# fallenshock/SinDDM

Measured on AMD Instinct MI355X. Metric: diffusion steps/sec (finest scale) + imgs/sec full multi-scale sample, 1/2/4/8 GPU, higher is better.
Workload: dtype f32 (3x3 convs: binary16 hi/lo split products -- Winograd-domain GEMMs with all 4 MFMA terms, fp32 accumulate; fp32-equivalent, error vs float64 = the fp32 oracle's: tests/test_gpu_h2.py; everything else fp32); 1 GPU; C3: 6-scale pyramid, T=1000, finest scale 411x512, batch 64 per GPU, dim=160; batch_per_gpu=64, global_batch=64, scale=5, parallelism=independent chains over 1 GPU(s), one all-gather of the images

## Files before the change

sinddm_amd/csrc/sinddm_fwd.hip:

```cpp
#include "conv_mfma.h"
#include "conv_wino4.h"
#include "conv_wh.h"
#include "internal.h"
#include "step_tail.h"
#include "chain_run.h"
#include <type_traits>
namespace sinddm {

ConvProfiler& conv_profiler() {
    static ConvProfiler p;
    return p;
}

__global__ void pack_kernel(const float* __restrict__ params, float* __restrict__ packed, PackArgs a) {
    long long i = (long long)blockIdx.x * blockDim.x + threadIdx.x;
    if (i >= a.total) return;
    int s = 0;
    long long base = 0;
    while (s < a.nseg - 1 && i >= base + a.seg[s].count) { base += a.seg[s].count; ++s; }
    const PackSeg& g = a.seg[s];
    const long long j = i - base;
    float v = 0.0f;
    if (g.kind == 0) {
        const int co_l = (int)(j % g.co_lds);
// ... 23 lines not shown
        const int cb = (int)r;
        const int m = cb * g.mt * 16 + mt * 16 + (lane & 15);
        const int k = ch * 16 + ks * 4 + (lane >> 4);
        const int M = g.transpose ? g.cin : g.cout;
        const int K = g.transpose ? g.cout : g.cin;
        if (m < M && k < K) {
            float gt[3][3];
#pragma unroll
            for (int a = 0; a < 3; ++a)
#pragma unroll
                for (int b2 = 0; b2 < 3; ++b2) {
                    const int tap = a * 3 + b2;
                    gt[a][b2] = g.transpose ? params[g.w + ((long long)k * g.cin + m) * 9 + (8 - tap)]
                                            : params[g.w + ((long long)m * g.cin + k) * 9 + tap];
                }
            const float G[4][3] = {{1.f, 0.f, 0.f}, {0.5f, 0.5f, 0.5f}, {0.5f, -0.5f, 0.5f}, {0.f, 0.f, 1.f}};
            const int fi = xi >> 2, fj = xi & 3;
            float acc = 0.f;
#pragma unroll
            for (int a = 0; a < 3; ++a) {
                float rowv = 0.f;
#pragma unroll
                for (int b2 = 0; b2 < 3; ++b2) rowv += G[fj][b2] * gt[a][b2];
                acc += G[fi][a] * rowv;
            }
            v = fi == 2 ? -acc : acc;
        }
    } else if (g.kind == 4) {
        long long r = j;
        const int slot = (int)(r % 4); r /= 4;
        const int lane = (int)(r % 64); r /= 64;
        const int q8 = (int)(r % 8); r /= 8;
        const int ks = (int)(r % 4); r /= 4;
        const int fi = (int)(r % 4); r /= 4;
        const int ch = (int)(r % g.nch); r /= g.nch;
        const int cb = (int)r;
        const int e = w3_pos_e(q8 * 4 + slot);
        const int mt = e < 0 ? 0 : e / 6, fj = e < 0 ? 0 : e - mt * 6;
        const int m = cb * 80 + mt * 16 + (lane & 15);
        const int k = ch * 16 + ks * 4 + (lane >> 4);
        const int M4 = g.transpose ? g.cin : g.cout, K4 = g.transpose ? g.cout : g.cin;
        if (e >= 0 && m < M4 && k < K4) {
            const double G2[4][3] = {{1., 0., 0.}, {.5, .5, .5}, {.5, -.5, .5}, {0., 0., 1.}};
            const double G4[6][3] = {{1. / 4, 0., 0.}, {-1. / 6, -1. / 6, -1. / 6}, {-1. / 6, 1. / 6, -1. / 6},
                                     {1. / 24, 1. / 12, 1. / 6}, {1. / 24, -1. / 12, 1. / 6}, {0., 0., 1.}};
            double acc = 0.;
#pragma unroll
            for (int a = 0; a < 3; ++a) {
                double rowv = 0.;
#pragma unroll
                for (int b2 = 0; b2 < 3; ++b2)
                    rowv += G4[fj][b2] * (double)(g.transpose ? params[g.w + ((long long)k * g.cin + m) * 9 + (2 - a) * 3 + (2 - b2)]
                                                              : params[g.w + ((long long)m * g.cin + k) * 9 + a * 3 + b2]);
                acc += G2[fi][a] * rowv;
            }
            v = (float)(fi == 2 ? -acc : acc);
        }
    } else if (g.kind == 1) {
        if (j < g.cout) {
            v = params[g.w + j];
            if (g.w2 >= 0) v += params[g.w2 + j];
        }
    }
    packed[g.dst + j] = v;
}

int pack_launch(const float* params, float* packed, const PackArgs& a, hipStream_t st) {
    const int threads = 256;
    const unsigned grid = (unsigned)((a.total + threads - 1) / threads);
    hipLaunchKernelGGL(pack_kernel, dim3(grid), dim3(threads), 0, st, params, packed, a);
    SINDDM_LAUNCH_CHECK();
    return 0;
}

static int pack_forward(const NetPlan& P, const float* params, float* packed, hipStream_t st) {
    PackArgs a{};
    auto add = [&](PackSeg s) { a.seg[a.nseg++] = s; a.total += s.count; };
    for (int l = 0; l < 4; ++l) {
        const BlockPlan& b = P.blk[l];
        pack_add_conv3x3(a, b.c1, 0, b.c1_w, 0);
        pack_add_conv3x3(a, b.c2, 0, b.c2_w, 0);
        if (b.nchr > 0) pack_add_direct(a, b.pk_res, b.res_w, b.cin, b.cout, 1, b.mt, b.coblks, 0);
        pack_add_conv3x3(a, b.c1, 3, b.c1_w, 0);
        pack_add_conv3x3(a, b.c2, 3, b.c2_w, 0);
        PackSeg t{};
        t.kind = 1; t.cout = b.cout; t.count = (long long)b.coblks * b.mt * 16;
        t.dst = b.pk_b1; t.w = b.c1_b; t.w2 = -1;
        add(t);
        t.dst = b.pk_b2; t.w = b.c2_b; t.w2 = b.res_b;
        add(t);
    }
    PackSeg z{};
    z.kind = 2; z.dst = P.pk_zero; z.count = 64;
    add(z);
    int rc = pack_launch(params, packed, a, st);
    if (rc) return rc;
    PackArgs f{};
    for (int l = 0; l < 4; ++l) {
        pack_add_conv3x3(f, P.blk[l].c1, 4, P.blk[l].c1_w, 0);
        pack_add_conv3x3(f, P.blk[l].c2, 4, P.blk[l].c2_w, 0);
    }
    if (f.nseg > 0) {
        rc = pack_launch(params, packed, f, st);
        if (rc) return rc;
    }
    for (int l = 0; l < 4; ++l) {
        rc = wh_pack(P.blk[l].c1, params + P.blk[l].c1_w, packed, 0, st);
        if (!rc) rc = wh_pack(P.blk[l].c2, params + P.blk[l].c2_w, packed, 0, st);
        if (rc) return rc;
    }
    return head_pack_launch(P, params, packed, st);
}

struct CondArgs {
    const float* params;
    const long long* t_dev;
    int t_host;
    int t_step;
    float scale;
    float* out;
    int cond_stride;
    long long tm0_w, tm0_b, tm2_w, tm2_b;
    long long mlp_w[4], mlp_b[4], tr_w[4], tr_b[4];
    int cin[4], coff[4];
    float* cond_vec;
    float* hidden;
    float* emb_out;
    float* mvec_out;
};
static CondArgs cond_args(const NetPlan& P, const float* params) {
    CondArgs ca{};
    ca.params = params; ca.cond_stride = P.cond_stride;
    ca.tm0_w = P.tm0_w; ca.tm0_b = P.tm0_b; ca.tm2_w = P.tm2_w; ca.tm2_b = P.tm2_b;
    for (int l = 0; l < 4; ++l) {
        ca.mlp_w[l] = P.blk[l].mlp_w; ca.mlp_b[l] = P.blk[l].mlp_b;
        ca.tr_w[l] = P.blk[l].tr_w; ca.tr_b[l] = P.blk[l].tr_b;
        ca.cin[l] = P.blk[l].cin; ca.coff[l] = P.blk[l].cond_off;
    }
    return ca;
}

__global__ __launch_bounds__(128) void cond_kernel(CondArgs a) {
    __shared__ float emb[64];
    __shared__ float h1[128];
    __shared__ float cv[32];
    __shared__ float gv[32];
    __shared__ float mv[32];
    const int b = blockIdx.x;
    const int tid = threadIdx.x;
    const float* P = a.params;
    const float tval = a.t_dev ? (float)a.t_dev[b] : (float)(a.t_host + b * a.t_step);
    if (tid < 32) {
        const int i = tid & 15;
        const float f = (float)exp((double)((float)i * -0.6140226914650789f));
        const float x = (tid < 16) ? tval : a.scale;
        const float arg = x * f;
        const int o = (tid < 16) ? 0 : 32;
        emb[o + i] = sinf(arg);
        emb[o + 16 + i] = cosf(arg);
    }
    __syncthreads();
    if (a.emb_out && tid < 64) a.emb_out[(long long)b * 64 + tid] = emb[tid];
    {
        float s = P[a.tm0_b + tid];
        const float* w = P + a.tm0_w + (long long)tid * 64;
#pragma unroll 8
        for (int k = 0; k < 64; ++k) s = fmaf(w[k], emb[k], s);
        if (a.hidden) a.hidden[(long long)b * 128 + tid] = s;
        h1[tid] = gelu_erf(s);
    }
    __syncthreads();
    if (tid < 32) {
        float s = P[a.tm2_b + tid];
        const float* w = P + a.tm2_w + (long long)tid * 128;
#pragma unroll 8
        for (int k = 0; k < 128; ++k) s = fmaf(w[k], h1[k], s);
        cv[tid] = s;
        gv[tid] = gelu_erf(s);
        if (a.cond_vec) a.cond_vec[(long long)b * 32 + tid] = s;
    }
    __syncthreads();
    for (int l = 0; l < 4; ++l) {
        if (tid < 32) {
            float s = P[a.mlp_b[l] + tid];
            const float* w = P + a.mlp_w[l] + (long long)tid * 32;
#pragma unroll 8
            for (int k = 0; k < 32; ++k) s = fmaf(w[k], gv[k], s);
            mv[tid] = s;
            if (a.mvec_out) a.mvec_out[((long long)b * 4 + l) * 32 + tid] = s;
        }
        __syncthreads();
        for (int c = tid; c < a.cin[l]; c += blockDim.x) {
            float s = P[a.tr_b[l] + c];
            const float* w = P + a.tr_w[l] + (long long)c * 32;
#pragma unroll 8
            for (int k = 0; k < 32; ++k) s = fmaf(w[k], mv[k], s);
            a.out[(long long)b * a.cond_stride + a.coff[l] + c] = s;
        }
        __syncthreads();
    }
}

#ifndef DW_RW_
#define DW_RW_ 4
#endif
constexpr int DW_RW = DW_RW_;
constexpr int DW_TH = 4 * DW_RW, DW_TW = 128, DW_RS = DW_TW + 4, DW_HR = DW_TH + 4;
#ifndef DW_NX_
#define DW_NX_ 2
#endif
constexpr int DW_NX = DW_NX_;

__global__ __launch_bounds__(256) void dwconv5_kernel(const float* __restrict__ x, const float* __restrict__ w,
                                                       const float* __restrict__ bias, const float* __restrict__ cond,
                                                       int cond_stride, const float* __restrict__ addt, int flip,
                                                       float* __restrict__ out, int C, int H, int W, int groupsX, int pi,
                                                       int po, float* __restrict__ amax) {
    __shared__ __attribute__((aligned(16))) float tile[DW_NX][DW_HR * DW_RS];
    const int c = blockIdx.y, b = blockIdx.z;
    const int ty = blockIdx.x / groupsX, gxi = blockIdx.x - ty * groupsX;
    const int y0 = ty * DW_TH, xg0 = gxi * (DW_NX * DW_TW);
    const size_t plane = ((size_t)b * C + c) * H * po;
    const float* src = x + ((size_t)b * C + c) * H * pi;
    constexpr int DW_GR = DW_RS / 4;
    constexpr int DW_NG = DW_HR * DW_GR;
    constexpr int DW_LD = (DW_NG + 255) / 256;
    const __amdgpu_buffer_rsrc_t rsx = __builtin_amdgcn_make_buffer_rsrc(const_cast<float*>(src), 0, H * pi * 4, 0x00020000);
    f32x4 stg[DW_NX][DW_LD];
#pragma unroll
    for (int t = 0; t < DW_NX; ++t) {
        const int x0 = xg0 + t * DW_TW;
#pragma unroll
        for (int k = 0; k < DW_LD; ++k) {
            const int i = threadIdx.x + k * 256;
            const int r = i / DW_GR, g = i - r * DW_GR;
            const int gy = y0 + r - 2, gx = x0 + 4 * g - 2;
            const bool rowok = i < DW_NG && x0 < W && gy >= 0 && gy < H;
            const bool left = gx < 0;
            const int off = rowok ? (gy * pi + (left ? 0 : gx)) * 4 : 0x40000000;
            const f32x4 q = __builtin_bit_cast(f32x4, __builtin_amdgcn_raw_buffer_load_b128(rsx, off, 0, 0));
            f32x4 v = left ? f32x4{0.f, 0.f, q[0], q[1]} : q;
#pragma unroll
            for (int e = 0; e < 4; ++e) v[e] = (rowok && gx + e < W) ? v[e] : 0.0f;
            stg[t][k] = v;
        }
    }
#pragma unroll
    for (int t = 0; t < DW_NX; ++t)
#pragma unroll
        for (int k = 0; k < DW_LD; ++k) {
            const int i = threadIdx.x + k * 256;
            if (i < DW_NG) *reinterpret_cast<f32x4*>(&tile[t][i * 4]) = stg[t][k];
        }
    float wk[25];
#pragma unroll
    for (int k = 0; k < 25; ++k) wk[k] = w[c * 25 + (flip ? 24 - k : k)];
    const float add = (bias ? bias[c] : 0.0f) + (cond ? cond[(size_t)b * cond_stride + c] : 0.0f);
    __syncthreads();
    const int lane = threadIdx.x & 63, wv = threadIdx.x >> 6;
    float mx = 0.f;
#pragma unroll
    for (int t = 0; t < DW_NX; ++t) {
        const int x0 = xg0 + t * DW_TW;
        if (x0 >= W) break;
        f32x2 o[DW_RW];
#pragma unroll
        for (int r = 0; r < DW_RW; ++r) o[r] = f32x2{add, add};
#pragma unroll
        for (int dy = 0; dy < DW_RW + 4; ++dy) {
            f32x2 v[5];
            const float* row = &tile[t][(wv * DW_RW + dy) * DW_RS + lane];
#pragma unroll
            for (int dx = 0; dx < 5; ++dx) v[dx] = f32x2{row[dx], row[dx + 64]};
#pragma unroll
            for (int r = 0; r < DW_RW; ++r) {
                const int ky = dy - r;
                if (ky >= 0 && ky < 5) {
#pragma unroll
                    for (int dx = 0; dx < 5; ++dx) o[r] += wk[ky * 5 + dx] * v[dx];
                }
            }
        }
#pragma unroll
        for (int h = 0; h < 2; ++h) {
            const int gx = x0 + lane + 64 * h;
            if (gx < po) {
#pragma unroll
                for (int r = 0; r < DW_RW; ++r) {
                    const int gy = y0 + wv * DW_RW + r;
                    if (gy < H) {
                        const size_t oidx = plane + (size_t)gy * po + gx;
                        const float ov = gx < W ? (addt ? o[r][h] + addt[oidx] : o[r][h]) : 0.0f;
                        mx = fmaxf(mx, fabsf(ov));
                        out[oidx] = ov;
                    }
                }
            }
        }
    }
    if (amax) amax_publish(mx, amax + (size_t)b * AMAX_STRIDE);
}

#ifndef DWR_ROWS_
#define DWR_ROWS_ 12
#endif
constexpr int DWR_ROWS = DWR_ROWS_;

__global__ __launch_bounds__(256) void dwconv5_rows_kernel(const float* __restrict__ x, const float* __restrict__ w,
                                                            const float* __restrict__ bias, const float* __restrict__ cond,
                                                            int cond_stride, const float* __restrict__ addt, int flip,
                                                            float* __restrict__ out, int C, int H, int W, int bandsX, int Wt,
                                                            float* __restrict__ amax) {
    const int c = blockIdx.y, b = blockIdx.z;
    const int by = blockIdx.x / bandsX, bx = blockIdx.x - by * bandsX;
    const int lane = threadIdx.x & 63, wv = threadIdx.x >> 6;
    const int x4 = (bx * 64 + lane) * 4;
    const int y0 = (by * 4 + wv) * DWR_ROWS;
    const size_t plane = ((size_t)b * C + c) * H * W;
    float wk[25];
#pragma unroll
    for (int k = 0; k < 25; ++k) wk[k] = w[c * 25 + (flip ? 24 - k : k)];
    const float add = (bias ? bias[c] : 0.0f) + (cond ? cond[(size_t)b * cond_stride + c] : 0.0f);
    if (y0 >= H) return;
    const __amdgpu_buffer_rsrc_t rsx = __builtin_amdgcn_make_buffer_rsrc(const_cast<float*>(x + plane), 0, H * W * 4, 0x00020000);
    constexpr int OOBI = 0x40000000;
    const bool colok = x4 < W;
    const bool lok = colok && x4 >= 4, rok = colok && x4 + 4 < W;
    f32x4 acc[DWR_ROWS];
#pragma unroll
    for (int r = 0; r < DWR_ROWS; ++r) acc[r] = f32x4{add, add, add, add};
#pragma unroll
    for (int ir = 0; ir < DWR_ROWS + 4; ++ir) {
        const int gy = y0 + ir - 2;
        const bool rowok = gy >= 0 && gy < H;
        const int base = (gy * W + x4) * 4;
        const f32x4 ql = __builtin_bit_cast(f32x4, __builtin_amdgcn_raw_buffer_load_b128(rsx, (rowok && lok) ? base - 16 : OOBI, 0, 0));
        const f32x4 qm = __builtin_bit_cast(f32x4, __builtin_amdgcn_raw_buffer_load_b128(rsx, (rowok && colok) ? base : OOBI, 0, 0));
        const f32x4 qr = __builtin_bit_cast(f32x4, __builtin_amdgcn_raw_buffer_load_b128(rsx, (rowok && rok) ? base + 16 : OOBI, 0, 0));
        const float in[8] = {ql[2], ql[3], qm[0], qm[1], qm[2], qm[3], qr[0], qr[1]};
#pragma unroll
        for (int r = 0; r < DWR_ROWS; ++r) {
            const int ky = ir - r;
            if (ky >= 0 && ky < 5) {
#pragma unroll
                for (int kx = 0; kx < 5; ++kx) {
#pragma unroll
                    for (int cc = 0; cc < 4; ++cc) acc[r][cc] = fmaf(wk[ky * 5 + kx], in[cc + kx], acc[r][cc]);
                }
            }
        }
    }
    float mx = 0.f;
#pragma unroll
    for (int r = 0; r < DWR_ROWS; ++r) {
        const int gy = y0 + r;
        if (colok && gy < H) {
            const size_t o = plane + (size_t)gy * W + x4;
            f32x4 v = acc[r];
            if (addt) v += *reinterpret_cast<const f32x4*>(addt + o);
            if (x4 + 4 > Wt) {
#pragma unroll
                for (int cc = 0; cc < 4; ++cc) v[cc] = x4 + cc < Wt ? v[cc] : 0.0f;
            }
            mx = fmaxf(fmaxf(mx, fmaxf(fabsf(v[0]), fabsf(v[1]))), fmaxf(fabsf(v[2]), fabsf(v[3])));
            *reinterpret_cast<f32x4*>(out + o) = v;
        }
    }
    if (amax) amax_publish(mx, amax + (size_t)b * AMAX_STRIDE);
}

#ifndef SINDDM_DW_ROWS
#define SINDDM_DW_ROWS 1
#endif

int dwconv_launch(const float* x, const float* w, const float* bias, const float* cond, int cond_stride,
                  const float* addt, int flip, float* out, int B, int C, int H, int W, hipStream_t st, int pi, int po,
                  float* amax) {
    if (pi <= 0) pi = W;
    if (po <= 0) po = W;
    if (SINDDM_DW_ROWS && pi % 4 == 0 && po == pi && pi >= 192) {
        const int bandsX = (pi + 255) / 256, bandsY = (H + 4 * DWR_ROWS - 1) / (4 * DWR_ROWS);
        hipLaunchKernelGGL(dwconv5_rows_kernel, dim3(bandsX * bandsY, C, B), dim3(256), 0, st, x, w, bias, cond, cond_stride,
                           addt, flip, out, C, H, pi, bandsX, W, amax);
        SINDDM_LAUNCH_CHECK();
        return 0;
    }
    const int tilesX = (W + DW_TW - 1) / DW_TW, tilesY = (H + DW_TH - 1) / DW_TH;
    const int groupsX = (tilesX + DW_NX - 1) / DW_NX;
    hipLaunchKernelGGL(dwconv5_kernel, dim3(groupsX * tilesY, C, B), dim3(256), 0, st, x, w, bias, cond, cond_stride,
                       addt, flip, out, C, H, W, groupsX, pi, po, amax);
    SINDDM_LAUNCH_CHECK();
    return 0;
}

__global__ __launch_bounds__(256) void conv3x3_c3_gelu_kernel(const float* __restrict__ in, const float* __restrict__ w,
                                                              const float* __restrict__ bias, float* __restrict__ out,
                                                              float* __restrict__ out_pre, int H, int W, int Cout,
                                                              int co_per_block, int Wt, float* __restrict__ amax) {
    const int HW = H * W;
    const int b = blockIdx.y;
    const int co0 = blockIdx.z * co_per_block;
    const int co1 = min(Cout, co0 + co_per_block);
    const int p = blockIdx.x * 256 + threadIdx.x;
    const bool live = p < HW;
    const int pc = live ? p : HW - 1;
    const int y = pc / W, x = pc - y * W;
    const float* src = in + (size_t)b * 3 * HW;
    float v[27];
#pragma unroll
    for (int ci = 0; ci < 3; ++ci)
#pragma unroll
        for (int ky = 0; ky < 3; ++ky)
#pragma unroll
            for (int kx = 0; kx < 3; ++kx) {
                const int gy = y + ky - 1, gx = x + kx - 1;
                const bool ok = gy >= 0 && gy < H && gx >= 0 && gx < W;
                v[ci * 9 + ky * 3 + kx] = ok ? src[(size_t)ci * HW + (size_t)gy * W + gx] : 0.0f;
            }
    float* dst = out + (size_t)b * Cout * HW + pc;
    float* dpre = out_pre ? out_pre + (size_t)b * Cout * HW + pc : nullptr;
    f32x2 vp[13];
#pragma unroll
    for (int j = 0; j < 13; ++j) vp[j] = f32x2{v[2 * j], v[2 * j + 1]};
    auto dot27 = [&](int co) __attribute__((always_inline)) -> float {
        const float* wc = w + co * 27;
        f32x2 acc2{bias[co], 0.f};
#pragma unroll
        for (int j = 0; j < 13; ++j) {
            const f32x2 wp{wc[2 * j], wc[2 * j + 1]};
            acc2 = __builtin_elementwise_fma(vp[j], wp, acc2);
        }
        return fmaf(v[26], wc[26], acc2.x + acc2.y);
    };
    int co = co0;
    float mx = 0.f;
#pragma unroll 2
    for (; co + 1 < co1; co += 2) {
        const f32x2 acc{dot27(co), dot27(co + 1)};
        if (live) {
            if (dpre) {
                dpre[(size_t)co * HW] = acc.x;
                dpre[(size_t)(co + 1) * HW] = acc.y;
            }
            const f32x2 g = gelu_erf2(acc);
            const float g0 = x < Wt ? g.x : 0.0f, g1 = x < Wt ? g.y : 0.0f;
            mx = fmaxf(mx, fmaxf(fabsf(g0), fabsf(g1)));
            dst[(size_t)co * HW] = g0;
            dst[(size_t)(co + 1) * HW] = g1;
        }
    }
    if (co < co1) {
        const float acc = dot27(co);
        if (live) {
            if (dpre) dpre[(size_t)co * HW] = acc;
            const float g0 = x < Wt ? gelu_erf(acc) : 0.0f;
            mx = fmaxf(mx, fabsf(g0));
            dst[(size_t)co * HW] = g0;
        }
    }
    if (amax) amax_publish(mx, amax + (size_t)b * AMAX_STRIDE);
}

__global__ __launch_bounds__(256) void pad_rows_kernel(const float* __restrict__ in, float* __restrict__ out, int H, int W,
                                                       int Wp, long long nrows) {
    const long long q = (long long)blockIdx.x * 256 + threadIdx.x;
    const int qpr = Wp >> 2;
    if (q >= nrows * qpr) return;
    const long long row = q / qpr;
    const int x = (int)(q - row * qpr) * 4;
    f32x4 v;
#pragma unroll
    for (int e = 0; e < 4; ++e) v[e] = x + e < W ? in[row * W + x + e] : 0.0f;
    *reinterpret_cast<f32x4*>(out + row * Wp + x) = v;
}
__global__ __launch_bounds__(256) void final_conv1x1_pitch_kernel(const float* __restrict__ a, const float* __restrict__ w,
                                                                  const float* __restrict__ bias, float* __restrict__ out,
                                                                  int C, int H, int W, int Wp) {
    const int b = blockIdx.y;
    const int qpr = Wp >> 2;
    const int q = blockIdx.x * 256 + threadIdx.x;
    if (q >= H * qpr) return;
    const int y = q / qpr, x = (q - y * qpr) * 4;
    const size_t HWp = (size_t)H * Wp;
    const float* src = a + (size_t)b * C * HWp + (size_t)y * Wp + x;
    f32x4 o0{bias[0], bias[0], bias[0], bias[0]}, o1{bias[1], bias[1], bias[1], bias[1]}, o2{bias[2], bias[2], bias[2], bias[2]};
#pragma unroll 8
    for (int c = 0; c < C; ++c) {
        const f32x4 v = *reinterpret_cast<const f32x4*>(src + (size_t)c * HWp);
        o0 += w[c] * v;
        o1 += w[C + c] * v;
        o2 += w[2 * C + c] * v;
    }
    const size_t HW = (size_t)H * W;
    float* dst = out + (size_t)b * 3 * HW + (size_t)y * W + x;
#pragma unroll
    for (int e = 0; e < 4; ++e) {
        if (x + e < W) {
            dst[e] = o0[e];
            dst[HW + e] = o1[e];
            dst[2 * HW + e] = o2[e];
        }
    }
}
__global__ __launch_bounds__(256) void final_conv1x1_kernel(const float* __restrict__ a, const float* __restrict__ w,
                                                            const float* __restrict__ bias, float* __restrict__ out,
                                                            int C, int HW) {
    const int b = blockIdx.y;
    const int p = (blockIdx.x * 256 + threadIdx.x) * 4;
    if (p >= HW) return;
    const float* src = a + (size_t)b * C * HW + p;
    float* dst = out + (size_t)b * 3 * HW + p;
    if (p + 3 < HW) {
        f32x4 o0{bias[0], bias[0], bias[0], bias[0]}, o1{bias[1], bias[1], bias[1], bias[1]},
            o2{bias[2], bias[2], bias[2], bias[2]};
#pragma unroll 8
        for (int c = 0; c < C; ++c) {
            const f32x4 v = *reinterpret_cast<const f32x4*>(src + (size_t)c * HW);
            o0 += w[c] * v;
            o1 += w[C + c] * v;
            o2 += w[2 * C + c] * v;
        }
        *reinterpret_cast<f32x4*>(dst) = o0;
        *reinterpret_cast<f32x4*>(dst + HW) = o1;
        *reinterpret_cast<f32x4*>(dst + 2 * (size_t)HW) = o2;
    } else {
        for (int j = 0; p + j < HW; ++j) {
            float o0 = bias[0], o1 = bias[1], o2 = bias[2];
            for (int c = 0; c < C; ++c) {
                const float v = src[(size_t)c * HW + j];
                o0 = fmaf(w[c], v, o0);
                o1 = fmaf(w[C + c], v, o1);
                o2 = fmaf(w[2 * C + c], v, o2);
            }
            dst[j] = o0;
            dst[HW + j] = o1;
            dst[2 * (size_t)HW + j] = o2;
        }
    }
}

enum { Q_FUSE_GX = 1,
       Q_FUSE_CAX = 2 };
enum { Q_ROUND_QUAD = 0, Q_ROUND_QUAD_UN4 = Q_FUSE_GX, Q_ROUND_FLOAT = Q_FUSE_GX | Q_FUSE_CAX };

__device__ __forceinline__ float q_fma(float a, float b, float c) { return __builtin_fmaf(a, b, c); }
__device__ __forceinline__ f32x4 q_fma(float a, f32x4 b, f32x4 c) { return __builtin_elementwise_fma(f32x4{a, a, a, a}, b, c); }

template <typename T>
__device__ __forceinline__ T q_sample_elem(const T& x, const T& o, const T& z, bool mix, float g, float ca, float cb, int r) {
    T v = x;
    if (mix) v = (r & Q_FUSE_GX) ? q_fma(g, v, (1.0f - g) * o) : q_fma(1.0f - g, o, g * v);
    return (r & Q_FUSE_CAX) ? q_fma(ca, v, cb * z) : q_fma(cb, z, ca * v);
}

template <int VEC, int UN>
__global__ __launch_bounds__(256) void q_sample_kernel(const float* __restrict__ x0, const float* __restrict__ xo,
                                                       const float* __restrict__ nz, float* __restrict__ out,
                                                       const float* __restrict__ tabA, const float* __restrict__ tabB,
                                                       const float* __restrict__ gam, const long long* __restrict__ t_dev,
                                                       int t_host, long long n) {
    const int b = blockIdx.y;
    const long long t = t_dev ? t_dev[b] : (long long)t_host;
    const float ca = tabA[t], cb = tabB[t];
    const float g = (xo != nullptr) ? gam[t] : 0.0f;
    const size_t base = (size_t)b * n;
    if constexpr (VEC == 4) {
        const long long nq = n >> 2;
        const f32x4* x4 = reinterpret_cast<const f32x4*>(x0 + base);
        const f32x4* o4 = xo ? reinterpret_cast<const f32x4*>(xo + base) : nullptr;
        const f32x4* z4 = reinterpret_cast<const f32x4*>(nz + base);
        f32x4* y4 = reinterpret_cast<f32x4*>(out + base);
        for (long long q0 = (long long)blockIdx.x * (256 * UN) + threadIdx.x; q0 < nq; q0 += (long long)gridDim.x * (256 * UN)) {
            f32x4 v[UN], z[UN], o[UN];
#pragma unroll
            for (int u = 0; u < UN; ++u) {
                const long long q = q0 + u * 256;
                const bool ok = q < nq;
                v[u] = ok ? __builtin_nontemporal_load(x4 + q) : f32x4{0.f, 0.f, 0.f, 0.f};
                z[u] = ok ? __builtin_nontemporal_load(z4 + q) : f32x4{0.f, 0.f, 0.f, 0.f};
                if (o4) o[u] = ok ? __builtin_nontemporal_load(o4 + q) : f32x4{0.f, 0.f, 0.f, 0.f};
            }
#pragma unroll
            for (int u = 0; u < UN; ++u) {
                const long long q = q0 + u * 256;
                if (q >= nq) continue;
                y4[q] = q_sample_elem(v[u], o[u], z[u], o4 != nullptr, g, ca, cb, UN == 4 ? Q_ROUND_QUAD_UN4 : Q_ROUND_QUAD);
            }
        }
    } else {
        for (long long i = (long long)blockIdx.x * 256 + threadIdx.x; i < n; i += (long long)gridDim.x * 256) {
            float o;
            if (xo) o = xo[base + i];
            out[base + i] = q_sample_elem(x0[base + i], o, nz[base + i], xo != nullptr, g, ca, cb, Q_ROUND_FLOAT);
        }
    }
}


template <bool WRAP>
__device__ __forceinline__ void upsample_axis(float scale, int dst, int n, int& i0, int& i1, float& lam) {
    float f = fmaf(scale, (float)dst + 0.5f, -0.5f);
    if (WRAP) {
        const float fl = floorf(f);
        lam = f - fl;
        i0 = (int)fl % n;
        if (i0 < 0) i0 += n;
        i1 = i0 + 1 == n ? 0 : i0 + 1;
    } else {
        f = f < 0.0f ? 0.0f : f;
        i0 = (int)f; if (i0 > n - 1) i0 = n - 1;
        i1 = i0 + 1 < n ? i0 + 1 : n - 1;
        lam = f - (float)i0;
    }
}

template <bool WRAP_Y, bool WRAP_X>
__global__ __launch_bounds__(256) void upsample_bilinear_kernel(const float* __restrict__ in, float* __restrict__ out,
                                                                int h, int w, int H, int W, float sy, float sx) {
    const int bc = blockIdx.y;
    const int p = blockIdx.x * 256 + threadIdx.x;
    if (p >= H * W) return;
    const int oy = p / W, ox = p - oy * W;
    int iy0, iy1, ix0, ix1;
    float ly, lx;
    upsample_axis<WRAP_Y>(sy, oy, h, iy0, iy1, ly);
    upsample_axis<WRAP_X>(sx, ox, w, ix0, ix1, lx);
    const float* s = in + (size_t)bc * h * w;
    const float tl = s[iy0 * w + ix0], tr = s[iy0 * w + ix1], bl = s[iy1 * w + ix0], br = s[iy1 * w + ix1];
    out[(size_t)bc * H * W + p] = (1.0f - ly) * ((1.0f - lx) * tl + lx * tr) + ly * ((1.0f - lx) * bl + lx * br);
}

template <int VEC>
__global__ __launch_bounds__(256) void wrap_halo_kernel(float* ext, const float* src, long long nq, int H, int W, int hy,
                                                        int hx) {
    const int He = H + 2 * hy, We = W + 2 * hx, qpr = We / VEC;
    for (long long q = (long long)blockIdx.x * 256 + threadIdx.x; q < nq; q += (long long)gridDim.x * 256) {
        const long long row = q / qpr;
        const int x = (int)(q - row * qpr) * VEC;
        const long long bc = row / He;
        const int y = (int)(row - bc * He);
        if (!src && y >= hy && y < hy + H && x >= hx && x < hx + W) continue;
        int cy = (y - hy) % H, cx = (x - hx) % W;
        if (cy < 0) cy += H;
        if (cx < 0) cx += W;
        const float* s = src ? src + ((size_t)bc * H + cy) * W + cx : ext + ((size_t)bc * He + hy + cy) * We + hx + cx;
        float* d = ext + ((size_t)bc * He + y) * We + x;
        if (VEC == 4) *reinterpret_cast<f32x4*>(d) = *reinterpret_cast<const f32x4*>(s);
        else *d = *s;
    }
}

int wrap_halo_launch(float* ext, const float* src, int BC, int H, int W, int hy, int hx, hipStream_t st) {
    if (hy == 0 && hx == 0 && !src) return 0;
    const bool vec = W % 4 == 0 && hx % 4 == 0 &&
                     ((reinterpret_cast<uintptr_t>(ext) | reinterpret_cast<uintptr_t>(src)) & 15) == 0;
    const long long nq = (long long)BC * (H + 2 * hy) * ((W + 2 * hx) / (vec ? 4 : 1));
    long long bx = (nq + 255) / 256;
    if (bx > 8192) bx = 8192;
    if (vec) hipLaunchKernelGGL(wrap_halo_kernel<4>, dim3((unsigned)bx), dim3(256), 0, st, ext, src, nq, H, W, hy, hx);
    else hipLaunchKernelGGL(wrap_halo_kernel<1>, dim3((unsigned)bx), dim3(256), 0, st, ext, src, nq, H, W, hy, hx);
    SINDDM_LAUNCH_CHECK();
    return 0;
}

template <int VEC>
__global__ __launch_bounds__(256) void q_sample_wrap_kernel(const float* __restrict__ x0, const float* __restrict__ xo,
                                                            const float* __restrict__ nz, float* __restrict__ ext,
// ... 1089 lines not shown
```

Before: 762.0 sample-steps/s (finest scale, batch x steps/s, all GPUs).

## Share depthwise conv halo across lanes via DPP and enlarge row band

The depthwise 5x5 row kernel now loads only the lane's own 16-byte chunk plus one 8-byte edge load (meaningful only at the wave's first and last lanes). Neighbour halo values come from adjacent lanes through DPP wave shifts, replacing three 128-bit loads per input row. Row bounds checks are folded into unsigned out-of-range buffer offsets, the wave index is made scalar, and rows per wave go from 12 to 16. The goal is less load traffic and fewer address instructions per row, at the cost of more registers for the larger accumulator array, which may reduce occupancy.

Measured after the change: 769.7 sample-steps/s (finest scale, batch x steps/s, all GPUs) (median of 6 runs). 1.01x the previous value.

```diff
diff --git a/sinddm_amd/csrc/sinddm_fwd.hip b/sinddm_amd/csrc/sinddm_fwd.hip
--- a/sinddm_amd/csrc/sinddm_fwd.hip
+++ b/sinddm_amd/csrc/sinddm_fwd.hip
@@ -349,9 +349,16 @@
 }
 
 #ifndef DWR_ROWS_
-#define DWR_ROWS_ 12
+#define DWR_ROWS_ 16
 #endif
 constexpr int DWR_ROWS = DWR_ROWS_;
+
+__device__ __forceinline__ float dpp_wave_shr1(float old, float src) {
+    return __builtin_bit_cast(float, __builtin_amdgcn_update_dpp(__builtin_bit_cast(int, old), __builtin_bit_cast(int, src), 0x138, 0xf, 0xf, false));
+}
+__device__ __forceinline__ float dpp_wave_shl1(float old, float src) {
+    return __builtin_bit_cast(float, __builtin_amdgcn_update_dpp(__builtin_bit_cast(int, old), __builtin_bit_cast(int, src), 0x130, 0xf, 0xf, false));
+}
 
 __global__ __launch_bounds__(256) void dwconv5_rows_kernel(const float* __restrict__ x, const float* __restrict__ w,
                                                             const float* __restrict__ bias, const float* __restrict__ cond,
@@ -360,7 +367,7 @@
                                                             float* __restrict__ amax) {
     const int c = blockIdx.y, b = blockIdx.z;
     const int by = blockIdx.x / bandsX, bx = blockIdx.x - by * bandsX;
-    const int lane = threadIdx.x & 63, wv = threadIdx.x >> 6;
+    const int lane = threadIdx.x & 63, wv = __builtin_amdgcn_readfirstlane(threadIdx.x >> 6);
     const int x4 = (bx * 64 + lane) * 4;
     const int y0 = (by * 4 + wv) * DWR_ROWS;
     const size_t plane = ((size_t)b * C + c) * H * W;
@@ -370,21 +377,21 @@
     const float add = (bias ? bias[c] : 0.0f) + (cond ? cond[(size_t)b * cond_stride + c] : 0.0f);
     if (y0 >= H) return;
     const __amdgpu_buffer_rsrc_t rsx = __builtin_amdgcn_make_buffer_rsrc(const_cast<float*>(x + plane), 0, H * W * 4, 0x00020000);
-    constexpr int OOBI = 0x40000000;
     const bool colok = x4 < W;
+    constexpr unsigned OOBV = 0x50000000u;
     const bool lok = colok && x4 >= 4, rok = colok && x4 + 4 < W;
+    const unsigned cm = colok ? (unsigned)x4 * 4u : OOBV;
+    const unsigned ce = lane == 0 ? (lok ? (unsigned)x4 * 4u - 8u : OOBV) : ((lane == 63 && rok) ? (unsigned)x4 * 4u + 16u : OOBV);
     f32x4 acc[DWR_ROWS];
 #pragma unroll
     for (int r = 0; r < DWR_ROWS; ++r) acc[r] = f32x4{add, add, add, add};
 #pragma unroll
     for (int ir = 0; ir < DWR_ROWS + 4; ++ir) {
-        const int gy = y0 + ir - 2;
-        const bool rowok = gy >= 0 && gy < H;
-        const int base = (gy * W + x4) * 4;
-        const f32x4 ql = __builtin_bit_cast(f32x4, __builtin_amdgcn_raw_buffer_load_b128(rsx, (rowok && lok) ? base - 16 : OOBI, 0, 0));
-        const f32x4 qm = __builtin_bit_cast(f32x4, __builtin_amdgcn_raw_buffer_load_b128(rsx, (rowok && colok) ? base : OOBI, 0, 0));
-        const f32x4 qr = __builtin_bit_cast(f32x4, __builtin_amdgcn_raw_buffer_load_b128(rsx, (rowok && rok) ? base + 16 : OOBI, 0, 0));
-        const float in[8] = {ql[2], ql[3], qm[0], qm[1], qm[2], qm[3], qr[0], qr[1]};
+        const unsigned ro = (unsigned)((y0 + ir - 2) * W) * 4u;
+        const f32x4 qm = __builtin_bit_cast(f32x4, __builtin_amdgcn_raw_buffer_load_b128(rsx, (int)(cm + ro), 0, 0));
+        const f32x2 qe = __builtin_bit_cast(f32x2, __builtin_amdgcn_raw_buffer_load_b64(rsx, (int)(ce + ro), 0, 0));
+        const float in[8] = {dpp_wave_shr1(qe[0], qm[2]), dpp_wave_shr1(qe[1], qm[3]), qm[0], qm[1], qm[2], qm[3],
+                             dpp_wave_shl1(qe[0], qm[0]), dpp_wave_shl1(qe[1], qm[1])};
 #pragma unroll
         for (int r = 0; r < DWR_ROWS; ++r) {
             const int ky = ir - r;
@@ -397,6 +404,7 @@
             }
         }
     }
+    const bool pads = bx * 256 + 256 > Wt;
     float mx = 0.f;
 #pragma unroll
     for (int r = 0; r < DWR_ROWS; ++r) {
@@ -405,11 +413,12 @@
             const size_t o = plane + (size_t)gy * W + x4;
             f32x4 v = acc[r];
             if (addt) v += *reinterpret_cast<const f32x4*>(addt + o);
-            if (x4 + 4 > Wt) {
+            if (pads) {
 #pragma unroll
                 for (int cc = 0; cc < 4; ++cc) v[cc] = x4 + cc < Wt ? v[cc] : 0.0f;
             }
-            mx = fmaxf(fmaxf(mx, fmaxf(fabsf(v[0]), fabsf(v[1]))), fmaxf(fabsf(v[2]), fabsf(v[3])));
+            mx = fmaxf(fmaxf(mx, fabsf(v[0])), fabsf(v[1]));
+            mx = fmaxf(fmaxf(mx, fabsf(v[2])), fabsf(v[3]));
             *reinterpret_cast<f32x4*>(out + o) = v;
         }
     }
```
